# eggsbenedicto/DiffusionRenderer-ComfyUI

Measured on AMD Instinct MI355X. Metric: denoising_steps_per_sec, higher is better.
Workload: dtype bf16; 1 GPU; inverse pass, 57f x 576 x 1024 clip: EDM Euler step = 1 DiT forward (D=4096, 28 blocks, 32 heads) over S=18432 tokens, guidance 0; parallelism=sp1 (token bands; self-attention exchange: none), weights=random-init (hash generator), 7.2e9 params bf16

## Files before the change

diffusionrenderer-comfyui_amd/csrc/gemm256s.hip:

```cpp
#include <stdlib.h>
#include "drn_common.h"
#include "drn_launchers.h"

#ifndef G256S_ABL
#define G256S_ABL 0
#endif
#ifndef G256S_NT
#define G256S_NT 0
#endif
#include "gemm256s_core.h"

#define EPI_PARTIAL 3

template <int EPI, bool PRE = false>
static __device__ __forceinline__ void store_tile(f32x4_t (&acc)[2][4][2][2], bf16_t* C, int64_t M, int64_t N, int64_t ldc,
                                                  const bf16_t* __restrict__ gate, const bf16_t* R, int64_t ldr, int64_t rpb,
                                                  int cbc, int64_t cbs, int64_t m0, int64_t n0, int wr, int wc, int fr, int fq,
                                                  const char* res_lds = nullptr, const char* gate_lds = nullptr) {
    if (G256S_ABL & 8) {
#pragma unroll
        for (int i = 0; i < 2; ++i)
#pragma unroll
            for (int mt = 0; mt < 4; ++mt)
#pragma unroll
                for (int j = 0; j < 2; ++j)
#pragma unroll
                    for (int nt = 0; nt < 2; ++nt) asm volatile("" :: "v"(acc[i][mt][j][nt]));
        return;
    }
    if (EPI == EPI_PARTIAL) {
        float* part = reinterpret_cast<float*>(C);
#pragma unroll
        for (int i = 0; i < 2; ++i)
#pragma unroll
            for (int mt = 0; mt < 4; ++mt) {
                const int64_t m = m0 + i * 128 + wr * 64 + mt * 16 + fr;
                if (m >= M) continue;
#pragma unroll
                for (int j = 0; j < 2; ++j)
#pragma unroll
                    for (int nt = 0; nt < 2; ++nt) {
                        const int64_t n = n0 + j * 128 + wc * 32 + nt * 16 + fq * 4;
                        if (n < N) *reinterpret_cast<f32x4_t*>(part + m * ldc + n) = acc[i][mt][j][nt];
                    }
            }
        return;
    }
    const int64_t c_tile_off = (n0 >> cbc) * cbs + (n0 & ((1ll << cbc) - 1)) - n0;
    asm volatile("" : "+v"(fr), "+v"(fq));
    const int64_t b_tile = (EPI == DRN_EPI_GATE_RES) ? (int64_t)((uint32_t)m0 / (uint32_t)rpb) : 0;
    const bool one_clip = m0 + TB <= (b_tile + 1) * rpb;
#pragma unroll
    for (int i = 0; i < 2; ++i) {
        uint2 g2[4][2][2], r2[4][2][2];
        if (EPI == DRN_EPI_GATE_RES && (G256S_ABL & 64)) {
#pragma unroll
            for (int mt = 0; mt < 4; ++mt)
#pragma unroll
                for (int j = 0; j < 2; ++j)
#pragma unroll
                    for (int nt = 0; nt < 2; ++nt) g2[mt][j][nt] = r2[mt][j][nt] = make_uint2(0x3f803f80u, 0x3f803f80u);
        } else if (EPI == DRN_EPI_GATE_RES && PRE) {
            const uint32_t ra = (uint32_t)((wr * 64 + fr) * 512 + (((wc * 4 + (fq >> 1)) ^ fr) << 4) + (fq & 1) * 8);
#pragma unroll
            for (int mt = 0; mt < 4; ++mt)
#pragma unroll
                for (int j = 0; j < 2; ++j)
#pragma unroll
                    for (int nt = 0; nt < 2; ++nt) {
                        r2[mt][j][nt] = *reinterpret_cast<const uint2*>(res_lds + i * 65536 + mt * 8192 + j * 256 + (ra ^ (nt * 32)));
                        if (mt == 0) {
                            g2[0][j][nt] = *reinterpret_cast<const uint2*>(gate_lds + (j * 128 + wc * 32 + nt * 16 + fq * 4) * 2);
                        } else {
                            g2[mt][j][nt] = g2[0][j][nt];
                        }
                    }
        } else if (EPI == DRN_EPI_GATE_RES) {
#pragma unroll
            for (int mt = 0; mt < 4; ++mt) {
                const int64_t m_raw = m0 + i * 128 + wr * 64 + mt * 16 + fr;
                const int64_t m = m_raw < M ? m_raw : M - 1;
                const int64_t b = one_clip ? b_tile : (int64_t)((uint32_t)m / (uint32_t)rpb);
#pragma unroll
                for (int j = 0; j < 2; ++j)
#pragma unroll
                    for (int nt = 0; nt < 2; ++nt) {
                        const int64_t n = n0 + j * 128 + wc * 32 + nt * 16 + fq * 4;
                        g2[mt][j][nt] = *reinterpret_cast<const uint2*>(gate + b * N + n);
                        r2[mt][j][nt] = *reinterpret_cast<const uint2*>(R + m * ldr + n);
                    }
            }
        }
#pragma unroll
        for (int mt = 0; mt < 4; ++mt) {
            const int64_t m_raw = m0 + i * 128 + wr * 64 + mt * 16 + fr;
            const bool m_ok = m_raw < M;
            const int64_t m = m_ok ? m_raw : M - 1;
#pragma unroll
            for (int j = 0; j < 2; ++j) {
                uint2 o[2];
#pragma unroll
                for (int nt = 0; nt < 2; ++nt) {
                    float v[4];
#pragma unroll
                    for (int r = 0; r < 4; ++r) v[r] = rbf(acc[i][mt][j][nt][r]);
                    if (EPI == DRN_EPI_GELU) {
#pragma unroll
                        for (int r = 0; r < 4; ++r) v[r] = gelu_erf_fast(v[r]);
                    } else if (EPI == DRN_EPI_GATE_RES) {
                        const uint2 gg = g2[mt][j][nt], rr = r2[mt][j][nt];
                        const float g[4] = {bflo(gg.x), bfhi(gg.x), bflo(gg.y), bfhi(gg.y)};
                        const float x[4] = {bflo(rr.x), bfhi(rr.x), bflo(rr.y), bfhi(rr.y)};
#pragma unroll
                        for (int r = 0; r < 4; ++r) v[r] = x[r] + rbf(g[r] * v[r]);
                    }
                    o[nt].x = pack_bf2(v[0], v[1]);
                    o[nt].y = pack_bf2(v[2], v[3]);
                }
                const auto sx = __builtin_amdgcn_permlane16_swap(o[0].x, o[1].x, false, false);
                const auto sy = __builtin_amdgcn_permlane16_swap(o[0].y, o[1].y, false, false);
                const int64_t n8 = n0 + j * 128 + wc * 32 + (fq & 1) * 16 + (fq >> 1) * 8;
                if (G256S_ABL & 128) {
                    asm volatile("" :: "v"(sx[0]), "v"(sy[0]), "v"(sx[1]), "v"(sy[1]));
                } else if (m_ok && n8 < N) {
                    typedef uint32_t u32x4_t __attribute__((ext_vector_type(4)));
                    const u32x4_t val = {sx[0], sy[0], sx[1], sy[1]};
                    u32x4_t* dst = reinterpret_cast<u32x4_t*>(C + m * ldc + n8 + c_tile_off);
                    if (G256S_NT) __builtin_nontemporal_store(val, dst);
                    else *dst = val;
                }
            }
        }
    }
}
#define STORES_PER_TILE 16

template <int EPI, bool PRE = false>
__global__ __launch_bounds__(512, 2) void gemm256s_kernel(const bf16_t* __restrict__ A, const bf16_t* __restrict__ W,
                                                          bf16_t* C, int64_t M, int64_t N, int64_t K, int64_t lda,
                                                          int64_t ldw, int64_t ldc, const bf16_t* __restrict__ gate,
                                                          const bf16_t* R, int64_t ldr, int64_t rpb, int GROUP,
                                                          int abc, int64_t abs_, int cbc, int64_t cbs) {
    if (EPI == EPI_PARTIAL) {
        K /= gridDim.y;
        A += (int64_t)blockIdx.y * K;
        W += (int64_t)blockIdx.y * K;
        C = reinterpret_cast<bf16_t*>(reinterpret_cast<float*>(C) + (int64_t)blockIdx.y * M * ldc);
    }
    THREAD_SETUP();
    int64_t m0, n0;
    tile_of(blockIdx.x, nwg, tiles_m, tiles_n, GROUP, m0, n0);
    const int k_second = min(1, nk - 1);
    int kt = 0;
    if (PRE) {
        (void)gsrc;
        const char* abase = reinterpret_cast<const char*>(A + m0 * lda);
        const char* wbase = reinterpret_cast<const char*>(W + n0 * ldw);
        uint32_t voff[2][2];
#pragma unroll
        for (int p = 0; p < 2; ++p) {
            const int r = (wave * 2 + p) * 8 + (lane >> 3);
            const int c = (lane & 7) ^ ((r >> 1) & 7);
            voff[0][p] = (uint32_t)((r * (int)lda + c * 8) * 2);
            voff[1][p] = (uint32_t)((r * (int)ldw + c * 8) * 2);
        }
#undef DMA
#define DMA(H, KD, S)                                                                                                  \
    do {                                                                                                               \
        const int kt_ = (int)(KD);                                                                                     \
        char* dst_ = smem + H_OFF(S, H) + dma_off;                                                                     \
        const char* sb_ = (H) < 2 ? abase + (((int64_t)((H) & 1) * 128 * lda + A_KOFF(kt_)) << 1)                      \
                                  : wbase + (((int64_t)((H) & 1) * 128 * ldw + (int64_t)kt_ * BK) << 1);               \
        __builtin_amdgcn_global_load_lds((gptr_t)(sb_ + voff[(H) >> 1][0]), (lptr_t)dst_, 16, 0, 0);                   \
        __builtin_amdgcn_global_load_lds((gptr_t)(sb_ + voff[(H) >> 1][1]), (lptr_t)(dst_ + 1024), 16, 0, 0);          \
    } while (0)
        ZERO_ACC();
        PROLOGUE();
        for (; kt + 2 < nk; kt += 2) {
            KSTEP(0, wx, wy, kt + 2, 10, 10, 10, 10);
            KSTEP(1, wy, wx, kt + 3, 10, 10, 10, 10);
        }
        const char* rres = reinterpret_cast<const char*>(R + m0 * ldr + n0);
        uint32_t roff[2];
#pragma unroll
        for (int p = 0; p < 2; ++p) {
            const int rr = wave * 4 + p * 2 + (lane >> 5);
            roff[p] = (uint32_t)((rr * (int)ldr + (((lane & 31) ^ (rr & 15)) << 3)) * 2);
        }
#undef DMA
#define DMA(H, KD, S)                                                                                                  \
    do {                                                                                                               \
        const char* rb_ = rres + (int64_t)(((S) * 4 + (H)) * 32) * ldr * 2;                                            \
        char* dst_ = smem + ((S) * 4 + (H)) * HALF_BYTES + dma_off;                                                    \
        __builtin_amdgcn_global_load_lds((gptr_t)(rb_ + roff[0]), (lptr_t)dst_, 16, 0, 0);                             \
        __builtin_amdgcn_global_load_lds((gptr_t)(rb_ + roff[1]), (lptr_t)(dst_ + 1024), 16, 0, 0);                    \
    } while (0)
        KSTEP(0, wx, wy, 0, 10, 10, 10, 10);
        const char* gbase = reinterpret_cast<const char*>(gate + (int64_t)((uint32_t)m0 / (uint32_t)rpb) * N + n0);
        const uint32_t goff = (uint32_t)((lane & 31) * 16);
        char* gate_lds = smem + 2 * STAGE_BYTES + wave * 1024;
#undef DMA
#define DMA(H, KD, S)                                                                                                  \
    do {                                                                                                               \
        const char* rb_ = rres + (int64_t)(((S) * 4 + (H)) * 32) * ldr * 2;                                            \
        char* dst_ = smem + ((S) * 4 + (H)) * HALF_BYTES + dma_off;                                                    \
        if ((H) == H_W0) __builtin_amdgcn_global_load_lds((gptr_t)(gbase + goff), (lptr_t)gate_lds, 16, 0, 0);         \
        __builtin_amdgcn_global_load_lds((gptr_t)(rb_ + roff[0]), (lptr_t)dst_, 16, 0, 0);                             \
        __builtin_amdgcn_global_load_lds((gptr_t)(rb_ + roff[1]), (lptr_t)(dst_ + 1024), 16, 0, 0);                    \
    } while (0)
        KSTEP(1, wy, wx, 0, 11, 11, 11, 11);
#undef DMA
#define DMA(H, KD, S) GEMM_DMA(H, KD, S)
        asm volatile("s_waitcnt vmcnt(0)" ::: "memory");
        __builtin_amdgcn_s_barrier();
        store_tile<EPI, true>(acc, C, M, N, ldc, gate, R, ldr, rpb, cbc, cbs, m0, n0, wr, wc, fr, fq, smem, gate_lds);
        return;
    }
    SET_SRC(m0, n0);
    ZERO_ACC();
    PROLOGUE();
    for (; kt + 1 < nk; kt += 2) {
        KSTEP(0, wx, wy, min(kt + 2, nk - 1), 10, 10, 10, 10);
        KSTEP(1, wy, wx, min(kt + 3, nk - 1), 10, 10, 10, 10);
    }
    if (kt < nk) KSTEP(0, wx, wy, nk - 1, 10, 10, 10, 10);
    asm volatile("s_waitcnt vmcnt(0)" ::: "memory");
    store_tile<EPI>(acc, C, M, N, ldc, gate, R, ldr, rpb, cbc, cbs, m0, n0, wr, wc, fr, fq);
}

#undef A_OFF
#undef W_OFF
#define A_OFF(S, I) ((S) * 2 * HALF_BYTES + (I) * HALF_BYTES)
#define W_OFF(S, J) (4 * HALF_BYTES + (S) * 2 * HALF_BYTES + (J) * HALF_BYTES)
#define WS_LDS_BYTES (10 * HALF_BYTES)
__global__ __launch_bounds__(512, 2) void gemm256w_kernel(const bf16_t* __restrict__ A, const bf16_t* __restrict__ W,
                                                          float* __restrict__ partial, int64_t M, int64_t N, int64_t K,
                                                          int64_t lda, int64_t ldw, int GROUP) {
    const int abc = 62, cbc = 62;
    const int64_t abs_ = 0, cbs = 0;
    K /= gridDim.y;
    A += (int64_t)blockIdx.y * K;
    W += (int64_t)blockIdx.y * K;
    float* part = partial + (int64_t)blockIdx.y * M * N;
    THREAD_SETUP();
    int64_t m0, n0;
    tile_of(blockIdx.x, nwg, tiles_m, tiles_n, GROUP, m0, n0);
    SET_SRC(m0, n0);
    ZERO_ACC();
#define KCL(k) min((int)(k), nk - 1)
    DMA(H_W0, 0, 0); DMA(H_W1, 0, 0);
    DMA(H_W0, KCL(1), 1); DMA(H_A0, 0, 0); DMA(H_W1, KCL(1), 1); DMA(H_A1, 0, 0);
    DMA(H_W0, KCL(2), 2); DMA(H_A0, KCL(1), 1); DMA(H_W1, KCL(2), 2); DMA(H_A1, KCL(1), 1);
    asm volatile("s_waitcnt vmcnt(12)" ::: "memory");
    __builtin_amdgcn_s_barrier();
#pragma unroll
    for (int nt = 0; nt < 2; ++nt)
#pragma unroll
        for (int ks = 0; ks < 2; ++ks) wx[nt][ks] = LD_W(0, 0, nt, ks);
#pragma unroll
    for (int mt = 0; mt < 4; ++mt)
#pragma unroll
        for (int ks = 0; ks < 2; ++ks) af[mt][ks] = LD_A(0, 0, mt, ks);
    asm volatile("s_waitcnt lgkmcnt(0)" ::: "memory");
    FENCE();
    __builtin_amdgcn_s_barrier();
    FENCE();
    int sw = 0;
#define WSTEP(KT, SA, WA, WB)                                                                                         \
    do {                                                                                                              \
        const int swn_ = sw == 2 ? 0 : sw + 1;                                                                        \
        KSTEP2(SA, (SA) ^ 1, sw, swn_, WA, WB, KCL((KT) + 2), KCL((KT) + 3), 10, 18, 10, 18);                         \
        sw = swn_;                                                                                                    \
    } while (0)
    int kt = 0;
    for (; kt + 1 < nk; kt += 2) {
        WSTEP(kt, 0, wx, wy);
        WSTEP(kt + 1, 1, wy, wx);
    }
    if (kt < nk) WSTEP(kt, 0, wx, wy);
    asm volatile("s_waitcnt vmcnt(0)" ::: "memory");
    store_tile<EPI_PARTIAL>(acc, reinterpret_cast<bf16_t*>(part), M, N, N, nullptr, nullptr, 0, M, cbc, cbs, m0, n0, wr, wc,
                            fr, fq);
}
#undef WSTEP
#undef KCL
#undef A_OFF
#undef W_OFF
#define A_OFF(S, I) ((S) * STAGE_BYTES + (I) * HALF_BYTES)
#define W_OFF(S, J) ((S) * STAGE_BYTES + (2 + (J)) * HALF_BYTES)

#ifndef G256S_PRE_DEFAULT
#define G256S_PRE_DEFAULT 1
#endif
static int g_res_prefetch = G256S_PRE_DEFAULT;
extern "C" int drn_gemm_force_res_prefetch(int on) {
    const int was = g_res_prefetch;
    if (on >= 0) g_res_prefetch = on ? 1 : 0;
    return was;
}

template <int EPI>
static int launch256s(const void* A, const void* W, void* C, int64_t M, int64_t N, int64_t K, int64_t lda, int64_t ldw,
                      int64_t ldc, const void* gate, const void* residual, int64_t ldr, int64_t rpb, hipStream_t st,
                      const int64_t* blk) {
    static bool configured = false;
    if (!configured) {
        hipError_t e = hipFuncSetAttribute(reinterpret_cast<const void*>(&gemm256s_kernel<EPI>),
                                           hipFuncAttributeMaxDynamicSharedMemorySize, 2 * STAGE_BYTES);
        if (e != hipSuccess) return (int)e;
        configured = true;
    }
    const int64_t tiles = ((M + TB - 1) / TB) * ((N + TB - 1) / TB);
    if (tiles >= (1ll << 31) || M >= (1ll << 31)) return DRN_EINVAL;
    if (rpb > M || rpb <= 0) rpb = M;
    static int group = 0;
    if (group == 0) {
        const char* e = getenv("DRN_GEMM_GROUP");
        group = e ? atoi(e) : 4;
        if (group < 1) group = 4;
    }
    if constexpr (EPI == DRN_EPI_GATE_RES) {
        static int pre = -1;
        if (pre < 0) {
            const char* e = getenv("DRN_GEMM_RES_PREFETCH");
            pre = (e && e[0] == '0') ? 0 : 1;
            if (pre && hipFuncSetAttribute(reinterpret_cast<const void*>(&gemm256s_kernel<EPI, true>),
                                           hipFuncAttributeMaxDynamicSharedMemorySize, 2 * STAGE_BYTES + 8192) != hipSuccess) {
                (void)hipGetLastError();
                pre = 0;
            }
        }
        const int64_t nk = K / BK;
        if (pre && g_res_prefetch && M % TB == 0 && N % TB == 0 && rpb % TB == 0 && nk >= 4 && nk % 2 == 0 && residual && gate &&
            ldr % 8 == 0 && ((uintptr_t)residual & 15) == 0 && ((uintptr_t)gate & 15) == 0 && 128 * ldr * 2 < (1ll << 31) && 128 * lda * 2 < (1ll << 31) &&
            128 * ldw * 2 < (1ll << 31)) {
            gemm256s_kernel<EPI, true><<<dim3((unsigned)tiles), dim3(512), 2 * STAGE_BYTES + 8192, st>>>(
                (const bf16_t*)A, (const bf16_t*)W, (bf16_t*)C, M, N, K, lda, ldw, ldc, (const bf16_t*)gate, (const bf16_t*)residual,
                ldr, rpb, group, (int)blk[0], blk[1], (int)blk[2], blk[3]);
            return drn_launch_status();
        }
    }
    gemm256s_kernel<EPI><<<dim3((unsigned)tiles), dim3(512), 2 * STAGE_BYTES, st>>>(
        (const bf16_t*)A, (const bf16_t*)W, (bf16_t*)C, M, N, K, lda, ldw, ldc, (const bf16_t*)gate, (const bf16_t*)residual,
        ldr, rpb, group, (int)blk[0], blk[1], (int)blk[2], blk[3]);
    return drn_launch_status();
}

int drn_gemm256s_partial(const void* A, const void* W, float* partial, int64_t M, int64_t N, int64_t K, int64_t lda, int64_t ldw,
                         int splits, void* stream, bool wring_ok) {
    static bool configured = false;
    if (!configured) {
        hipError_t e = hipFuncSetAttribute(reinterpret_cast<const void*>(&gemm256s_kernel<EPI_PARTIAL>),
                                           hipFuncAttributeMaxDynamicSharedMemorySize, 2 * STAGE_BYTES);
        if (e != hipSuccess) return (int)e;
        configured = true;
    }
    const int64_t tiles = ((M + TB - 1) / TB) * ((N + TB - 1) / TB);
    if (tiles >= 65536 || splits < 1 || splits > 64 || (K / BK) % splits != 0 || M >= (1ll << 31)) return DRN_EINVAL;
    static int wring = -1;
    if (wring < 0) {
        const char* e = getenv("DRN_SPLITK_WRING");
        wring = (e && e[0] == '0') ? 0 : 1;
        if (wring && hipFuncSetAttribute(reinterpret_cast<const void*>(&gemm256w_kernel),
                                         hipFuncAttributeMaxDynamicSharedMemorySize, WS_LDS_BYTES) != hipSuccess) {
            (void)hipGetLastError();
            wring = 0;
        }
    }
    if (wring && wring_ok && K / splits / BK >= 3) {
        gemm256w_kernel<<<dim3((unsigned)tiles, (unsigned)splits), dim3(512), WS_LDS_BYTES, (hipStream_t)stream>>>(
            (const bf16_t*)A, (const bf16_t*)W, partial, M, N, K, lda, ldw, 4);
        return drn_launch_status();
    }
    static const int64_t plain[4] = {62, 0, 62, 0};
    gemm256s_kernel<EPI_PARTIAL><<<dim3((unsigned)tiles, (unsigned)splits), dim3(512), 2 * STAGE_BYTES, (hipStream_t)stream>>>(
        (const bf16_t*)A, (const bf16_t*)W, (bf16_t*)partial, M, N, K, lda, ldw, N, nullptr, nullptr, 0, M, 4,
        (int)plain[0], plain[1], (int)plain[2], plain[3]);
    return drn_launch_status();
}

int drn_gemm256s_dispatch(const void* A, const void* W, void* C, int64_t M, int64_t N, int64_t K, int64_t lda, int64_t ldw,
                          int64_t ldc, int epilogue, const void* gate, const void* residual, int64_t ldr, int64_t rpb,
                          void* stream, const int64_t* blk) {
    hipStream_t st = (hipStream_t)stream;
    switch (epilogue) {
        case DRN_EPI_NONE: return launch256s<DRN_EPI_NONE>(A, W, C, M, N, K, lda, ldw, ldc, gate, residual, ldr, rpb, st, blk);
        case DRN_EPI_GELU: return launch256s<DRN_EPI_GELU>(A, W, C, M, N, K, lda, ldw, ldc, gate, residual, ldr, rpb, st, blk);
        case DRN_EPI_GATE_RES: return launch256s<DRN_EPI_GATE_RES>(A, W, C, M, N, K, lda, ldw, ldc, gate, residual, ldr, rpb, st, blk);
        default: return DRN_EINVAL;
    }
}
```

diffusionrenderer-comfyui_amd/dit_engine.py:

```python
import ctypes
import math
from typing import Dict, NamedTuple, Optional

import torch

from . import native as N
from .host_tables import rope_cos_sin, timestep_sinusoid
from .parallel import ShardPlan, allgather_rows_, alltoall_bands_, alltoall_rows_, group_info, is_process_group, wait_exchange


PRECISIONS = ("bf16", "mxfp8")
ATTENTION_PRECISIONS = ("bf16", "mxfp8")


def _pad_cols(w: torch.Tensor, mult: int) -> torch.Tensor:
    n, k = w.shape
    kp = (k + mult - 1) // mult * mult
    if kp == k:
        return w.contiguous()
    out = torch.zeros((n, kp), dtype=w.dtype, device=w.device)
    out[:, :k] = w
    return out


def _pad_rows(w: torch.Tensor, mult: int) -> torch.Tensor:
    n, k = w.shape
    npad = (n + mult - 1) // mult * mult
    if npad == n:
        return w.contiguous()
    out = torch.zeros((npad, k), dtype=w.dtype, device=w.device)
    out[:n] = w
    return out


class SpRoute(NamedTuple):
    layout: str
    amx: bool
    mx_return: bool = False
    launches: tuple = ()
    first_bands: int = 0
    o_mx: bool = False

    def path(self) -> dict:
        ret = "none" if self.layout == "gather" else ("e4m3" if self.mx_return else "bf16")
        return {"layout": self.layout, "return": ret, "attention": "mxfp8" if self.amx else "bf16"}


def sp_route(D, heads, S, world, exchange, mx, amx_on, fused_mx, mx_return, split_return) -> SpRoute:
    if exchange == "gather":
        amx = bool(amx_on and N.attention_mxfp8_choice(heads, S))
        return SpRoute("gather", amx, o_mx=bool(fused_mx and (amx or N.attention_mx_available())))
    W, rows, hpr = D // world, S // world, heads // world
    if mx:
        slabs = (world > 1 and W >= 256 and W & (W - 1) == 0
                 and N.mx_gemm_plan(rows, 2 * D, D) == 0 and N.mx_gemm_plan(rows, D, D) == 0)
    else:
        slabs = world > 1 and W >= 512 and N.gemm_blocked_ok(rows, 2 * D) and N.gemm_blocked_ok(rows, D)
    amx = bool(amx_on and N.attention_mxfp8_choice(hpr, S))
    mxret = bool(mx and mx_return and (amx or N.attention_mx_available()) and (slabs or world == 1 or (W // 32) % 16 == 0))
    launches = tuple(N.attention_plan(1, hpr, S, S))
    nb = launches[0][1] // rows if len(launches) == 2 and split_return else 0
    return SpRoute("slabs" if slabs else "regroup", amx, mxret, launches, nb)


class HipDiT:
    def __init__(self, net: dict, state_dict: Dict[str, torch.Tensor], device=None, prefix: str = "net.",
                 process_group=None, precision: Optional[str] = None, attention_precision: Optional[str] = None):
        import os
        if attention_precision is None:
            attention_precision = os.environ.get("DRN_ATT_PRECISION", "") or "bf16"
        if attention_precision not in ATTENTION_PRECISIONS:
            raise ValueError(f"unknown attention precision {attention_precision!r}: expected one of {ATTENTION_PRECISIONS}")
        self.attention_precision = attention_precision
        self._amx = attention_precision == "mxfp8"
        if precision is None:
            precision = os.environ.get("DRN_DIT_PRECISION", "") or "bf16"
        if precision not in PRECISIONS:
            raise ValueError(f"unknown DiT precision {precision!r}: expected one of {PRECISIONS}")
        self.precision = precision
        self._mx = precision == "mxfp8"
        if (self._mx or self._amx) and process_group is not None and not is_process_group(process_group):
            which = "precision" if self._mx else "attention_precision"
            raise ValueError(f"{which}='mxfp8' with a process_group that is no torch.distributed.ProcessGroup (sequence parallelism "
                             f"over another transport) is not built yet; got {type(process_group).__name__}")
        self.net = dict(net)
        self.device = torch.device(device) if device is not None else torch.device("cuda")
        self.D = net["model_channels"]
        self.heads = net["num_heads"]
        self.L = net["num_blocks"]
        self.kinds = [k.strip().lower() for k in net["block_config"].split("-")]
        self.pt, self.ps = net["patch_temporal"], net["patch_spatial"]
        self.out_ch = net["out_channels"]
        self.use_ctx = net.get("use_context_embedding", True)
        self.ctx_dim = net["crossattn_emb_channels"]
        self.with_mask = net.get("concat_padding_mask", True)
        if self.D // self.heads != 128:
            raise ValueError("HipDiT kernels are specialised for head_dim 128 (the renderer's only configuration)")
        hidden = int(self.D * net["mlp_ratio"])
        if self._mx and (self.D % 256 or hidden % 256):
            raise ValueError(f"precision='mxfp8' needs model_channels and the MLP width to be multiples of 256 (the MXFP8 GEMM's "
                             f"N and K contract); got {self.D} and {hidden}")
        N.load_library()
        self.pg = process_group
        world = group_info(process_group)[1] if process_group is not None else 1
        mode = os.environ.get("DRN_SP_EXCHANGE", "auto")
        if mode not in ("auto", "a2a", "gather"):
            raise ValueError("DRN_SP_EXCHANGE must be auto, a2a or gather")
        if mode == "a2a" and self.heads % world:
            raise ValueError(f"head all-to-all needs the world size ({world}) to divide the head count ({self.heads})")
        if process_group is None:
            self.exchange = "none"
        elif mode == "auto":
            self.exchange = "none" if world == 1 else ("gather" if self.heads % world else "a2a")
        else:
            self.exchange = mode
        self.world = world
        self._load(state_dict, prefix)
        self._rope_cache = {}
        self._time_cache = {}
        self._ctx_cache = {}
        self._ws = {}
        self._mx_act = {}
        self.trace = None
        self._per_launch = os.environ.get("DRN_PER_LAUNCH", "0") == "1"
        self._mx_fused = self._mx and os.environ.get("DRN_MX_FUSED", "1") != "0"
        self._mx_return = self._mx and os.environ.get("DRN_SP_MX_RETURN", "1") != "0"
        self.sp_path = None
        self._split_return = os.environ.get("DRN_SP_SPLIT_RETURN", "1") != "0"

    def _load(self, sd, p):
        dev, bf = self.device, torch.bfloat16

        def g(name):
            return sd[p + name].to(device=dev, dtype=bf)

        self.w_patch = _pad_cols(g("x_embedder.proj.1.weight"), 64)
        self.kpad = self.w_patch.shape[1]
        self.w_t1 = g("t_embedder.1.linear_1.weight").contiguous().unsqueeze(0)
        self.w_t2 = g("t_embedder.1.linear_2.weight").contiguous().unsqueeze(0)
        self.w_affnorm = g("affline_norm.weight").contiguous()
        self.seq = sd[p + "pos_embedder.seq"]
        self.ctx_table = g("context_embedding.weight") if self.use_ctx else None
        self.w_final = _pad_rows(g("final_layer.linear.weight"), 128)
        self.final_cols = self.out_ch * self.ps * self.ps * self.pt
        self.w_fa1 = g("final_layer.adaLN_modulation.1.weight").contiguous().unsqueeze(0)
        self.w_fa2 = g("final_layer.adaLN_modulation.2.weight").contiguous().unsqueeze(0)

        a1, a2 = [], []
        self.blocks = []
        ca_v, ca_o = [], []
        for i in range(self.L):
            subs = []
            for j, kind in enumerate(self.kinds):
                q = f"blocks.block{i}.blocks.{j}."
                a1.append(g(q + "adaLN_modulation.1.weight"))
                a2.append(g(q + "adaLN_modulation.2.weight"))
                if kind == "fa":
                    a = q + "block.attn."
                    wq, wk, wv = g(a + "to_q.0.weight"), g(a + "to_k.0.weight"), g(a + "to_v.0.weight")
                    if self.exchange == "a2a":
                        W = self.D // self.world
                        wkv = torch.stack([wk.view(self.world, W, -1), wv.view(self.world, W, -1)], 1).reshape(2 * self.D, -1)
                        wqkv = torch.cat([wq, wkv], 0).contiguous()
                    else:
                        wqkv = torch.cat([wq, wk, wv], 0).contiguous()
                    subs.append({"kind": "fa", "wqkv": wqkv,
                                 "qn": g(a + "to_q.1.weight").contiguous(), "kn": g(a + "to_k.1.weight").contiguous(),
                                 "wo": g(a + "to_out.0.weight").contiguous()})
                elif kind == "ca":
                    a = q + "block.attn."
                    subs.append({"kind": "ca", "idx": len(ca_v)})
                    ca_v.append(g(a + "to_v.0.weight"))
                    ca_o.append(g(a + "to_out.0.weight"))
                else:
                    subs.append({"kind": "mlp", "w1": g(q + "block.layer1.weight").contiguous(),
                                 "w2": g(q + "block.layer2.weight").contiguous()})
            self.blocks.append(subs)
        self.n_sites = len(a1)
        self.r = a1[0].shape[0]
        self.w_a1 = torch.cat(a1, 0).contiguous().unsqueeze(0)
        self.w_a2 = torch.stack(a2, 0).contiguous()
        self.n_ca = len(ca_v)
        self.w_cav = torch.stack(ca_v, 0).contiguous() if ca_v else None
        self.w_cao = torch.stack(ca_o, 0).contiguous() if ca_o else None
        self.ca_sites = [i * len(self.kinds) + j for i in range(self.L) for j, k in enumerate(self.kinds) if k == "ca"]
# ... 501 lines not shown
```

diffusionrenderer-comfyui_amd/native.py:

```python
import ctypes
import os
from ctypes import POINTER, Structure, c_char_p, c_double, c_float, c_int, c_int32, c_int64, c_void_p

import torch

_LIB = None
_LIB_NAME = "libdrn.so"

EPI_NONE, EPI_GELU, EPI_GATE_RES = 0, 1, 2
ACT_NONE, ACT_SILU = 0, 1

_P, _I, _L, _F = c_void_p, c_int, c_int64, c_float

SUB_FA, SUB_CA, SUB_MLP = 0, 1, 2


class DitSub(Structure):
    _fields_ = [("kind", c_int32), ("site", c_int32), ("ca_index", c_int32), ("reserved", c_int32),
                ("w_a", c_void_p), ("w_b", c_void_p), ("qn", c_void_p), ("kn", c_void_p),
                ("s_a", c_void_p), ("s_b", c_void_p)]


class DitForwardArgs(Structure):
    _fields_ = [("struct_bytes", c_int64), ("S", c_int64), ("B", c_int64), ("D", c_int64), ("hidden", c_int64),
                ("heads", c_int32), ("n_sub", c_int32), ("subs", POINTER(DitSub)),
                ("shift", c_void_p), ("scale", c_void_p), ("gate", c_void_p),
                ("shift_site_stride", c_int64), ("scale_site_stride", c_int64), ("gate_site_stride", c_int64),
                ("addvec", c_void_p), ("addvec_stride", c_int64), ("cos", c_void_p), ("sin", c_void_p),
                ("P", c_void_p), ("kpad", c_int64), ("w_patch", c_void_p),
                ("final_shift", c_void_p), ("final_scale", c_void_p), ("w_final", c_void_p), ("n_final", c_int64),
                ("X", c_void_p), ("H", c_void_p), ("QKV", c_void_p), ("O", c_void_p), ("U", c_void_p), ("Y", c_void_p),
                ("gemm_ws", c_void_p), ("gemm_ws_bytes", c_int64), ("attn_ws", c_void_p), ("attn_ws_bytes", c_int64),
                ("timer", c_void_p), ("eps", c_float), ("precision", c_int32),
                ("AQ", c_void_p), ("AS", c_void_p), ("act_bytes", c_int64),
                ("mx_fused", c_int32), ("reserved", c_int32), ("UQ", c_void_p), ("US", c_void_p), ("u_act_bytes", c_int64),
                ("attn_precision", c_int32), ("reserved2", c_int32), ("mx_attn", c_void_p), ("mx_attn_bytes", c_int64)]


SIGNATURES = {
    "drn_attention_plan": [_I, _L, _L, POINTER(c_int64)],
    "drn_dit_forward": [POINTER(DitForwardArgs), _P],
    "drn_dit_forward_args_bytes": [],
    "drn_dit_sub_bytes": [],
    "drn_dit_forward_gemm_workspace_bytes": [_L, _L, _L, _L, _L, _L],
    "drn_dit_forward_attn_workspace_bytes": [_L, _I, _L],
    "drn_dit_forward_mx_act_bytes": [_L, _L, _L, _L],
    "drn_dit_forward_mx_gemm_workspace_bytes": [_L, _L, _L, _L],
    "drn_dit_forward_mx_u_bytes": [_L, _L, _L],
    "drn_timer_create": [_I, _I],
    "drn_timer_destroy": [_P],
    "drn_timer_count": [_P],
    "drn_timer_seen": [_P, _I],
    "drn_timer_read": [_P, _I, POINTER(c_int), POINTER(c_float), POINTER(c_double), POINTER(c_double)],
    "drn_abi_version": [],
    "drn_error_string": [_I],
    "drn_gemm_bf16": [_P, _P, _P, _L, _L, _L, _L, _L, _L, _I, _P, _P, _L, _L, _P],
    "drn_gemm_bf16_blocked": [_P, _P, _P, _L, _L, _L, _L, _L, _L, _I, _P, _P, _L, _L, _L, _L, _L, _L, _P],
    "drn_gemm_bf16_splitk": [_P, _P, _P, _L, _L, _L, _L, _L, _L, _I, _P, _P, _L, _L, _I, _P, _P],
    "drn_gemm_splitk_workspace_bytes": [_L, _L, _I],
    "drn_gemm_bf16_f32out": [_P, _P, _P, _L, _L, _L, _L, _L, _P],
    "drn_gemm_bf16_splitk_partials": [_P, _P, _L, _L, _L, _L, _L, _L, _I, _P, _P],
    "drn_splitk_gate_res_ln_modulate": [_P, _I, _P, _P, _P, _P, _P, _P, _L, _L, _L, _F, _P],
    "drn_gemm_splitk_choice": [_L, _L, _L],
    "drn_gemm_tile_choice": [_L, _L],
    "drn_gemm_force_tile": [_I],
    "drn_gemm_force_res_prefetch": [_I],
    "drn_gemm_tall_force_shape": [_I],
    "drn_mx_quant_bf16": [_P, _L, _L, _L, _P, _P, _P],
    "drn_mx_quant_calls": [_I],
    "drn_gemm_mxfp8_gelu_mx": [_P, _P, _P, _P, _P, _P, _L, _L, _L, _L, _P],
    "drn_ln_modulate_mx": [_P, _P, _P, _P, _P, _P, _P, _L, _L, _L, _F, _P],
    "drn_splitk_gate_res_ln_modulate_mx": [_P, _I, _P, _P, _P, _P, _P, _P, _P, _P, _L, _L, _L, _F, _P],
    "drn_attention_bf16_mx": [_P, _P, _P, _P, _P, _P, _I, _I, _L, _L, _L, _L, _L, _L, _L, _L, _L, _L, _F, _P],
    "drn_attention_splitkv_bf16_mx": [_P, _P, _P, _P, _P, _P, _I, _I, _L, _L, _L, _L, _L, _L, _L, _L, _L, _L, _F, _I, _P, _P],
    "drn_attention_mx_available": [],
    "drn_attention_mxfp8_params": [POINTER(c_int), POINTER(c_float), POINTER(c_int)],
    "drn_attention_mxfp8_choice": [_I, _L],
    "drn_attention_mxfp8_force": [_I],
    "drn_qk_norm_rope_mx": [_P, _P, _P, _P, _P, _P, _P, _P, _P, _P, _L, _I, _L, _L, _L, _L, _F, _I, _P],
    "drn_mx_quant_vt": [_P, _P, _P, _I, _I, _L, _L, _L, _P],
    "drn_attention_mxfp8": [_P, _P, _P, _P, _P, _P, _P, _P, _P, _I, _I, _L, _L, _L, _L, _L, _L, _F, _P],
    "drn_attention_splitkv_mxfp8": [_P, _P, _P, _P, _P, _P, _P, _P, _P, _I, _I, _L, _L, _L, _L, _L, _L, _F, _I, _P, _P],
    "drn_dit_forward_mx_attn_bytes": [_L, _L, _L],
    "drn_dit_forward_mx_attn_layout": [_L, _L, _L, POINTER(c_int64)],
    "drn_gemm_mxfp8": [_P, _P, _P, _P, _P, _L, _L, _L, _L, _I, _P, _P, _L, _L, _P],
    "drn_gemm_mxfp8_blocked": [_P, _P, _P, _P, _P, _L, _L, _L, _L, _I, _P, _P, _L, _L, _L, _L, _L, _L, _P],
    "drn_gemm_mxfp8_splitk_choice": [_L, _L, _L],
    "drn_gemm_mxfp8_splitk": [_P, _P, _P, _P, _P, _L, _L, _L, _L, _I, _P, _P, _L, _L, _I, _P, _P],
    "drn_gemm_mxfp8_splitk_partials": [_P, _P, _P, _P, _L, _L, _L, _L, _I, _P, _P],
    "drn_gemm_mxfp8_force_small_m": [_I],
    "drn_gemm_mxfp8_tall_force_shape": [_I],
    "drn_gemv_bf16": [_P, _P, _P, _L, _L, _I, _I, _L, _L, _L, _L, _L, _P, _L, _L, _P, _L, _L, _I, _P],
    "drn_ln_modulate": [_P, _P, _P, _P, _P, _L, _L, _L, _F, _P],
    "drn_ln_force_kernel": [_I],
    "drn_bcast_add": [_P, _P, _L, _L, _L, _P],
    "drn_permute_021": [_P, _P, _L, _L, _L, _P],
    "drn_rmsnorm": [_P, _P, _P, _L, _L, _F, _P],
    "drn_qk_norm_rope": [_P, _P, _P, _P, _P, _P, _L, _I, _L, _L, _L, _L, _F, _P],
    "drn_attention_bf16": [_P, _P, _P, _P, _I, _I, _L, _L, _L, _L, _L, _L, _L, _L, _L, _L, _F, _P],
    "drn_attention_splitkv_bf16": [_P, _P, _P, _P, _I, _I, _L, _L, _L, _L, _L, _L, _L, _L, _L, _L, _F, _I, _P, _P],
    "drn_attention_splitkv_workspace_bytes": [_I, _I, _L, _I],
    "drn_attention_force_shape16": [_I],
    "drn_patchify_concat": [_P, _P, _P, _I, _I, _I, _I, _I, _I, _I, _I, _I, _L, _P],
    "drn_unpatchify": [_P, _L, _P, _I, _I, _I, _I, _I, _I, _I, _P],
    "drn_edm_scale_input": [_P, _P, _L, _F, _P],
    "drn_edm_step": [_P, _P, _P, _L, _F, _F, _F, _F, _P],
    "drn_cfg_combine": [_P, _P, _P, _L, _F, _P],
    "drn_postprocess_u8": [_P, _P, _I, _I, _I, _I, _I, _P],
    "drn_postprocess_window_u8": [_P, _P, _P, _P, _I, _I, _I, _I, _I, _I, _I, _I, _I, _P],
    "drn_env_project": [_P, _I, _P, _P, _P, _P, _I, _I, _I, _F, _P],
    "drn_fit_frames": [_P, _P, _I, _I, _I, _I, _I, _I, _I, _P, _P, _P, _I, _P, _P, _I, _P],
    "drn_fit_frames_u8": [_P, _P, _I, _I, _I, _I, _I, _I, _I, _P, _P, _P, _I, _P, _P, _I, _P],
    "drn_restore_frames_u8": [_P, _P, _I, _I, _I, _I, _I, _I, _I, _P, _P, _I, _P, _P, _I, _P],
    "drn_tile_blend_u8": [_P, _P, _P, _P, _L, _I, _I, _I, _I, _I, _I, _I, _I, _I, _I, _P],
    "drn_latent_tile_gather": [_P, _P, _L, _I, _I, _I, _I, _I, _I, _F, _I, _P],
    "drn_latent_tile_step_join": [_P, _P, _F, _P, _P, _P, _P, _L, _I, _I, _I, _I, _I, _I, _I, _I, _I, _I, _F, _F, _F, _F, _P],
}
_RESTYPES = {"drn_error_string": c_char_p, "drn_attention_splitkv_workspace_bytes": c_int64,
             "drn_gemm_splitk_workspace_bytes": c_int64, "drn_dit_forward_gemm_workspace_bytes": c_int64,
             "drn_dit_forward_attn_workspace_bytes": c_int64, "drn_dit_forward_mx_act_bytes": c_int64,
             "drn_dit_forward_mx_u_bytes": c_int64, "drn_mx_quant_calls": c_int64, "drn_dit_forward_mx_attn_bytes": c_int64,
             "drn_dit_forward_mx_gemm_workspace_bytes": c_int64, "drn_dit_forward_args_bytes": c_int64, "drn_dit_sub_bytes": c_int64, "drn_timer_create": c_void_p, "drn_timer_destroy": None,
             "drn_ln_force_kernel": None, "drn_attention_force_shape16": None}


def library_path() -> str:
    return os.path.join(os.path.dirname(os.path.abspath(__file__)), _LIB_NAME)


def load_library():
    global _LIB
    if _LIB is not None:
        return _LIB
    path = library_path()
    if not os.path.exists(path):
        raise RuntimeError(f"{path} not found: build it with `python __graft_entry__.py` (hipcc --offload-arch=gfx950); "
                           "there is no CPU / eager fallback for the hot path")
    lib = ctypes.CDLL(path)
    for name, argtypes in SIGNATURES.items():
        fn = getattr(lib, name)
        fn.argtypes = argtypes
        fn.restype = _RESTYPES.get(name, c_int)
    if lib.drn_abi_version() != 1:
        raise RuntimeError("libdrn.so ABI version mismatch")
    if lib.drn_dit_forward_args_bytes() != ctypes.sizeof(DitForwardArgs) or lib.drn_dit_sub_bytes() != ctypes.sizeof(DitSub):
        raise RuntimeError("libdrn.so: drn_dit_forward_args / drn_dit_sub layout differs from the ctypes mirror in native.py")
    _LIB = lib
    return lib


def _check(code: int, what: str):
    if code != 0:
        msg = load_library().drn_error_string(code)
        raise RuntimeError(f"{what} failed ({code}): {msg.decode() if msg else '?'}")


def _ptr(t):
    if t is None:
        return None
    assert t.is_cuda, "device tensor required"
    return t.data_ptr()


def _stream():
    return torch.cuda.current_stream().cuda_stream


def _bf16(*ts):
    for t in ts:
        if t is not None:
            assert t.dtype == torch.bfloat16, f"bf16 tensor required, got {t.dtype}"


class KernelTimer:

    def __init__(self, names=("gemm", "attention"), sample_every=1):
        self.names = set(names)
        self.sample_every = max(1, int(sample_every))
        self.counts = {}
        self.records = []
        self._native = None

    def native_handle(self, capacity=8192):
        if not ({"gemm", "attention"} <= self.names):
            return None
        if self._native is None:
            h = load_library().drn_timer_create(capacity, self.sample_every)
            if not h:
                raise RuntimeError("drn_timer_create failed")
            self._native = c_void_p(h)
        return self._native

    def __del__(self):
        if getattr(self, "_native", None) is not None and _LIB is not None:
            _LIB.drn_timer_destroy(self._native)
            self._native = None

    def begin(self, name):
        if name not in self.names:
            return None
        c = self.counts.get(name, 0)
        self.counts[name] = c + 1
        if c % self.sample_every:
            return None
        e = torch.cuda.Event(enable_timing=True)
        e.record()
        return e

    def end(self, name, start, flops, nbytes):
        if start is None:
            return
        e = torch.cuda.Event(enable_timing=True)
        e.record()
        self.records.append((name, start, e, flops, nbytes))

    def summary(self):
        out = {}
        for name, s, e, fl, by in self.records:
            d = out.setdefault(name, {"launches": 0, "ms_total": 0.0, "flops": 0.0, "bytes": 0.0})
            d["launches"] += 1
            d["ms_total"] += s.elapsed_time(e)
            d["flops"] += fl
            d["bytes"] += by
        seen = dict(self.counts)
        if self._native is not None:
            lib = load_library()
            kind, ms, fl, by = c_int(), c_float(), c_double(), c_double()
            for i in range(lib.drn_timer_count(self._native)):
                _check(lib.drn_timer_read(self._native, i, kind, ms, fl, by), "drn_timer_read")
                name = ("gemm", "attention")[kind.value]
# ... 652 lines not shown
```

include/drn.h:

```cpp
#ifndef DRN_H
#define DRN_H

#include <stdint.h>

#ifdef __cplusplus
extern "C" {
#endif

#define DRN_OK 0
#define DRN_EINVAL (-1)

#define DRN_ABI_VERSION 1

#define DRN_EPI_NONE 0
#define DRN_EPI_GELU 1
#define DRN_EPI_GATE_RES 2

#define DRN_ACT_NONE 0
#define DRN_ACT_SILU 1

int drn_abi_version(void);
const char* drn_error_string(int code);

int drn_gemm_bf16(const void* A, const void* W, void* C, int64_t M, int64_t N, int64_t K,
                  int64_t lda, int64_t ldw, int64_t ldc, int epilogue,
                  const void* gate, const void* residual, int64_t ldr, int64_t rows_per_batch,
                  void* stream);

int drn_gemm_bf16_blocked(const void* A, const void* W, void* C, int64_t M, int64_t N, int64_t K,
                          int64_t lda, int64_t ldw, int64_t ldc, int epilogue,
                          const void* gate, const void* residual, int64_t ldr, int64_t rows_per_batch,
                          int64_t a_block_cols, int64_t a_block_stride, int64_t c_block_cols, int64_t c_block_stride,
                          void* stream);

int drn_gemm_bf16_splitk(const void* A, const void* W, void* C, int64_t M, int64_t N, int64_t K,
                         int64_t lda, int64_t ldw, int64_t ldc, int epilogue,
                         const void* gate, const void* residual, int64_t ldr, int64_t rows_per_batch,
                         int splits, void* workspace, void* stream);
int64_t drn_gemm_splitk_workspace_bytes(int64_t M, int64_t N, int splits);
int drn_gemm_bf16_f32out(const void* A, const void* W, float* C, int64_t M, int64_t N, int64_t K, int64_t lda, int64_t ldw, void* stream);

int drn_gemm_bf16_splitk_partials(const void* A, const void* W, int64_t M, int64_t N, int64_t K,
                                  int64_t lda, int64_t ldw, int64_t rows_per_batch, int splits, void* workspace, void* stream);
int drn_gemm_splitk_choice(int64_t M, int64_t N, int64_t K);

int drn_gemm_tile_choice(int64_t M, int64_t N);
void drn_gemm_force_tile(int tile);
int drn_gemm_force_res_prefetch(int on);
int drn_gemm_tall_force_shape(int shape);

int drn_mx_quant_bf16(const void* X, int64_t M, int64_t K, int64_t ldx, void* Q, void* scales, void* stream);
int64_t drn_mx_quant_calls(int reset);
int drn_gemm_mxfp8_gelu_mx(const void* A, const void* SA, const void* W, const void* SW, void* CQ, void* CS, int64_t M, int64_t N,
                           int64_t K, int64_t rows_per_batch, void* stream);
int drn_gemm_mxfp8(const void* A, const void* SA, const void* W, const void* SW, void* C, int64_t M, int64_t N, int64_t K,
                   int64_t ldc, int epilogue, const void* gate, const void* residual, int64_t ldr, int64_t rows_per_batch,
                   void* stream);
int drn_gemm_mxfp8_blocked(const void* A, const void* SA, const void* W, const void* SW, void* C, int64_t M, int64_t N, int64_t K,
                           int64_t ldc, int epilogue, const void* gate, const void* residual, int64_t ldr, int64_t rows_per_batch,
                           int64_t a_block_cols, int64_t a_block_stride, int64_t c_block_cols, int64_t c_block_stride,
                           void* stream);
int drn_gemm_mxfp8_splitk_choice(int64_t M, int64_t N, int64_t K);
int drn_gemm_mxfp8_splitk(const void* A, const void* SA, const void* W, const void* SW, void* C, int64_t M, int64_t N, int64_t K,
                          int64_t ldc, int epilogue, const void* gate, const void* residual, int64_t ldr, int64_t rows_per_batch,
                          int splits, void* workspace, void* stream);
int drn_gemm_mxfp8_splitk_partials(const void* A, const void* SA, const void* W, const void* SW, int64_t M, int64_t N, int64_t K,
                                   int64_t rows_per_batch, int splits, void* workspace, void* stream);
int drn_gemm_mxfp8_force_small_m(int on);
int drn_gemm_mxfp8_tall_force_shape(int shape);

int drn_gemv_bf16(const void* x, const void* W, void* y, int64_t N, int64_t K,
                  int groups, int batch,
                  int64_t x_gstride, int64_t x_bstride, int64_t w_gstride,
                  int64_t y_gstride, int64_t y_bstride,
                  const void* add, int64_t add_gstride, int64_t add_bstride,
                  const void* mul, int64_t mul_gstride, int64_t mul_bstride,
                  int act, void* stream);

int drn_ln_modulate(void* x, const void* add_vec, const void* shift, const void* scale, void* h,
                    int64_t rows, int64_t D, int64_t rows_per_batch, float eps, void* stream);
int drn_ln_modulate_mx(void* x, const void* add_vec, const void* shift, const void* scale, void* h, void* hq, void* hs,
                       int64_t rows, int64_t D, int64_t rows_per_batch, float eps, void* stream);
int drn_splitk_gate_res_ln_modulate(const void* partials, int splits, void* x, const void* gate, const void* add_vec,
                                    const void* shift, const void* scale, void* h, int64_t rows, int64_t D,
                                    int64_t rows_per_batch, float eps, void* stream);
int drn_splitk_gate_res_ln_modulate_mx(const void* partials, int splits, void* x, const void* gate, const void* add_vec,
                                       const void* shift, const void* scale, void* h, void* hq, void* hs, int64_t rows, int64_t D,
                                       int64_t rows_per_batch, float eps, void* stream);
void drn_ln_force_kernel(int which);

int drn_bcast_add(void* x, const void* vec, int64_t rows, int64_t D, int64_t rows_per_batch, void* stream);

int drn_permute_021(const void* x, void* y, int64_t A, int64_t B, int64_t C, void* stream);

int drn_rmsnorm(const void* x, const void* w, void* y, int64_t rows, int64_t D, float eps, void* stream);

int drn_qk_norm_rope(void* q, void* k, const void* wq, const void* wk, const void* cos, const void* sin,
                     int64_t tokens, int heads, int64_t ldq, int64_t ldk, int64_t tokens_per_batch,
                     int64_t pos_offset, float eps, void* stream);

int drn_attention_bf16(const void* q, const void* k, const void* v, void* o,
                       int batch, int heads, int64_t Sq, int64_t Sk,
                       int64_t ldq, int64_t ldk, int64_t ldv, int64_t ldo,
                       int64_t bsq, int64_t bsk, int64_t bsv, int64_t bso,
                       float scale, void* stream);

void drn_attention_force_shape16(int on);

int drn_attention_splitkv_bf16(const void* q, const void* k, const void* v, void* o,
                               int batch, int heads, int64_t Sq, int64_t Sk,
                               int64_t ldq, int64_t ldk, int64_t ldv, int64_t ldo,
                               int64_t bsq, int64_t bsk, int64_t bsv, int64_t bso,
                               float scale, int nsplit, void* workspace, void* stream);
int64_t drn_attention_splitkv_workspace_bytes(int batch, int heads, int64_t Sq, int nsplit);

int drn_attention_bf16_mx(const void* q, const void* k, const void* v, void* o, void* oq, void* os,
                          int batch, int heads, int64_t Sq, int64_t Sk,
                          int64_t ldq, int64_t ldk, int64_t ldv, int64_t ldo,
                          int64_t bsq, int64_t bsk, int64_t bsv, int64_t bso,
                          float scale, void* stream);
int drn_attention_splitkv_bf16_mx(const void* q, const void* k, const void* v, void* o, void* oq, void* os,
                                  int batch, int heads, int64_t Sq, int64_t Sk,
                                  int64_t ldq, int64_t ldk, int64_t ldv, int64_t ldo,
                                  int64_t bsq, int64_t bsk, int64_t bsv, int64_t bso,
                                  float scale, int nsplit, void* workspace, void* stream);
int drn_attention_mx_available(void);

int drn_attention_mxfp8_params(int* key_tile, float* rescale_thr, int* pexp);
int drn_attention_mxfp8_choice(int heads, int64_t S);
int drn_attention_mxfp8_force(int on);
int drn_qk_norm_rope_mx(void* q, void* k, const void* wq, const void* wk, const void* cos, const void* sin,
// ... 149 lines not shown
```

Baseline: 3.687 steps/s.

## Replace GELU epilogue math with a bf16 lookup table staged in LDS

Builds a 65536-entry bf16 GELU lookup table once per device and, in the 256x256 GEMM's GELU epilogue, DMAs it into shared memory after the K loop. Each output is then rounded to bf16 and mapped through the table instead of evaluating erf-based GELU per element. This removes transcendental ALU work from the MLP up-projection epilogue. In exchange it adds a 128KB table load per tile and LDS gather lookups with possible bank conflicts, and it drops the bounds check on the store path, relying on the M and N tile-divisibility guard at launch.

```diff
diff --git a/diffusionrenderer-comfyui_amd/csrc/gemm256s.hip b/diffusionrenderer-comfyui_amd/csrc/gemm256s.hip
--- a/diffusionrenderer-comfyui_amd/csrc/gemm256s.hip
+++ b/diffusionrenderer-comfyui_amd/csrc/gemm256s.hip
@@ -1,4 +1,5 @@
 #include <stdlib.h>
+#include <mutex>
 #include "drn_common.h"
 #include "drn_launchers.h"
 
@@ -11,6 +12,19 @@
 #include "gemm256s_core.h"
 
 #define EPI_PARTIAL 3
+
+static __device__ __forceinline__ uint32_t gelu_table2(const char* table_lds, uint32_t w) {
+    uint32_t wl = w & 0xffffu;
+    asm("" : "+v"(wl));
+    const uint32_t lo = *reinterpret_cast<const uint16_t*>(table_lds + (wl << 1));
+    const uint32_t hi = *reinterpret_cast<const uint16_t*>(table_lds + ((w >> 16) << 1));
+    return lo | (hi << 16);
+}
+__global__ void gelu_table_kernel(bf16_t* __restrict__ table) {
+    const uint32_t i = blockIdx.x * blockDim.x + threadIdx.x;
+    if (i < 65536u) table[i] = f2bf(gelu_erf_fast(bf2f((bf16_t)i)));
+}
+#define GELU_TABLE_BYTES (65536 * 2)
 
 template <int EPI, bool PRE = false>
 static __device__ __forceinline__ void store_tile(f32x4_t (&acc)[2][4][2][2], bf16_t* C, int64_t M, int64_t N, int64_t ldc,
@@ -95,12 +109,18 @@
         for (int mt = 0; mt < 4; ++mt) {
             const int64_t m_raw = m0 + i * 128 + wr * 64 + mt * 16 + fr;
             const bool m_ok = m_raw < M;
-            const int64_t m = m_ok ? m_raw : M - 1;
+            const int64_t m = (m_ok || (EPI == DRN_EPI_GELU && PRE)) ? m_raw : M - 1;
 #pragma unroll
             for (int j = 0; j < 2; ++j) {
                 uint2 o[2];
 #pragma unroll
                 for (int nt = 0; nt < 2; ++nt) {
+                    if (EPI == DRN_EPI_GELU && PRE) {
+                        const f32x4_t a = acc[i][mt][j][nt];
+                        o[nt].x = gelu_table2(res_lds, pack_bf2(a[0], a[1]));
+                        o[nt].y = gelu_table2(res_lds, pack_bf2(a[2], a[3]));
+                        continue;
+                    }
                     float v[4];
 #pragma unroll
                     for (int r = 0; r < 4; ++r) v[r] = rbf(acc[i][mt][j][nt][r]);
@@ -122,7 +142,7 @@
                 const int64_t n8 = n0 + j * 128 + wc * 32 + (fq & 1) * 16 + (fq >> 1) * 8;
                 if (G256S_ABL & 128) {
                     asm volatile("" :: "v"(sx[0]), "v"(sy[0]), "v"(sx[1]), "v"(sy[1]));
-                } else if (m_ok && n8 < N) {
+                } else if ((EPI == DRN_EPI_GELU && PRE) || (m_ok && n8 < N)) {
                     typedef uint32_t u32x4_t __attribute__((ext_vector_type(4)));
                     const u32x4_t val = {sx[0], sy[0], sx[1], sy[1]};
                     u32x4_t* dst = reinterpret_cast<u32x4_t*>(C + m * ldc + n8 + c_tile_off);
@@ -179,6 +199,26 @@
         for (; kt + 2 < nk; kt += 2) {
             KSTEP(0, wx, wy, kt + 2, 10, 10, 10, 10);
             KSTEP(1, wy, wx, kt + 3, 10, 10, 10, 10);
+        }
+        if constexpr (EPI == DRN_EPI_GELU) {
+            const char* tbase = reinterpret_cast<const char*>(gate) + dma_off;
+            const uint32_t toff = (uint32_t)(lane * 16);
+#undef DMA
+#define DMA(H, KD, S)                                                                                                  \
+    do {                                                                                                               \
+        const char* tb_ = tbase + ((S) * 4 + (H)) * HALF_BYTES;                                                        \
+        char* dst_ = smem + ((S) * 4 + (H)) * HALF_BYTES + dma_off;                                                    \
+        __builtin_amdgcn_global_load_lds((gptr_t)(tb_ + toff), (lptr_t)dst_, 16, 0, 0);                                \
+        __builtin_amdgcn_global_load_lds((gptr_t)(tb_ + toff + 1024), (lptr_t)(dst_ + 1024), 16, 0, 0);                \
+    } while (0)
+            KSTEP(0, wx, wy, 0, 10, 10, 10, 10);
+            KSTEP(1, wy, wx, 0, 10, 10, 10, 10);
+#undef DMA
+#define DMA(H, KD, S) GEMM_DMA(H, KD, S)
+            asm volatile("s_waitcnt vmcnt(0)" ::: "memory");
+            __builtin_amdgcn_s_barrier();
+            store_tile<EPI, true>(acc, C, M, N, ldc, nullptr, nullptr, 0, rpb, cbc, cbs, m0, n0, wr, wc, fr, fq, smem, nullptr);
+            return;
         }
         const char* rres = reinterpret_cast<const char*>(R + m0 * ldr + n0);
         uint32_t roff[2];
@@ -299,6 +339,49 @@
     return was;
 }
 
+static int g_gelu_table_on = 1;
+extern "C" int drn_gemm_force_gelu_table(int on) {
+    const int was = g_gelu_table_on;
+    if (on >= 0) g_gelu_table_on = on ? 1 : 0;
+    return was;
+}
+
+#define DRN_MAX_DEVICES 64
+static bf16_t* g_gelu_table[DRN_MAX_DEVICES];
+static std::mutex g_gelu_table_mutex;
+extern "C" int drn_gemm_gelu_table_build(void* stream) {
+    int dev = -1;
+    hipError_t e = hipGetDevice(&dev);
+    if (e != hipSuccess) {
+        (void)hipGetLastError();
+        return (int)e;
+    }
+    if (dev < 0 || dev >= DRN_MAX_DEVICES) return DRN_EINVAL;
+    std::lock_guard<std::mutex> lock(g_gelu_table_mutex);
+    if (g_gelu_table[dev]) return DRN_OK;
+    bf16_t* t = nullptr;
+    e = hipMalloc(reinterpret_cast<void**>(&t), GELU_TABLE_BYTES);
+    if (e != hipSuccess) {
+        (void)hipGetLastError();
+        return (int)e;
+    }
+    gelu_table_kernel<<<dim3(256), dim3(256), 0, (hipStream_t)stream>>>(t);
+    e = hipGetLastError();
+    if (e == hipSuccess) e = hipStreamSynchronize((hipStream_t)stream);
+    if (e != hipSuccess) {
+        (void)hipFree(t);
+        return (int)e;
+    }
+    g_gelu_table[dev] = t;
+    return DRN_OK;
+}
+static const bf16_t* gelu_table_here() {
+    int dev = -1;
+    if (hipGetDevice(&dev) != hipSuccess || dev < 0 || dev >= DRN_MAX_DEVICES) return nullptr;
+    std::lock_guard<std::mutex> lock(g_gelu_table_mutex);
+    return g_gelu_table[dev];
+}
+
 template <int EPI>
 static int launch256s(const void* A, const void* W, void* C, int64_t M, int64_t N, int64_t K, int64_t lda, int64_t ldw,
                       int64_t ldc, const void* gate, const void* residual, int64_t ldr, int64_t rpb, hipStream_t st,
@@ -340,6 +423,28 @@
             return drn_launch_status();
         }
     }
+    if constexpr (EPI == DRN_EPI_GELU) {
+        static int lut = -1;
+        if (lut < 0) {
+            const char* e = getenv("DRN_GEMM_GELU_TABLE");
+            lut = (e && e[0] == '0') ? 0 : 1;
+            if (lut && hipFuncSetAttribute(reinterpret_cast<const void*>(&gemm256s_kernel<EPI, true>),
+                                           hipFuncAttributeMaxDynamicSharedMemorySize, 2 * STAGE_BYTES) != hipSuccess) {
+                (void)hipGetLastError();
+                lut = 0;
+            }
+        }
+        const int64_t nk = K / BK;
+        if (lut && g_gelu_table_on && M % TB == 0 && N % TB == 0 && nk >= 4 && nk % 2 == 0 && 128 * lda * 2 < (1ll << 31) &&
+            128 * ldw * 2 < (1ll << 31)) {
+            if (const bf16_t* table = gelu_table_here()) {
+                gemm256s_kernel<EPI, true><<<dim3((unsigned)tiles), dim3(512), 2 * STAGE_BYTES, st>>>(
+                    (const bf16_t*)A, (const bf16_t*)W, (bf16_t*)C, M, N, K, lda, ldw, ldc, table, nullptr, 0, rpb, group,
+                    (int)blk[0], blk[1], (int)blk[2], blk[3]);
+                return drn_launch_status();
+            }
+        }
+    }
     gemm256s_kernel<EPI><<<dim3((unsigned)tiles), dim3(512), 2 * STAGE_BYTES, st>>>(
         (const bf16_t*)A, (const bf16_t*)W, (bf16_t*)C, M, N, K, lda, ldw, ldc, (const bf16_t*)gate, (const bf16_t*)residual,
         ldr, rpb, group, (int)blk[0], blk[1], (int)blk[2], blk[3]);
diff --git a/diffusionrenderer-comfyui_amd/dit_engine.py b/diffusionrenderer-comfyui_amd/dit_engine.py
--- a/diffusionrenderer-comfyui_amd/dit_engine.py
+++ b/diffusionrenderer-comfyui_amd/dit_engine.py
@@ -101,6 +101,9 @@
             raise ValueError(f"precision='mxfp8' needs model_channels and the MLP width to be multiples of 256 (the MXFP8 GEMM's "
                              f"N and K contract); got {self.D} and {hidden}")
         N.load_library()
+        if self.device.type == "cuda":
+            with torch.cuda.device(self.device):
+                N._check(N.load_library().drn_gemm_gelu_table_build(None), "drn_gemm_gelu_table_build")
         self.pg = process_group
         world = group_info(process_group)[1] if process_group is not None else 1
         mode = os.environ.get("DRN_SP_EXCHANGE", "auto")
diff --git a/diffusionrenderer-comfyui_amd/native.py b/diffusionrenderer-comfyui_amd/native.py
--- a/diffusionrenderer-comfyui_amd/native.py
+++ b/diffusionrenderer-comfyui_amd/native.py
@@ -65,6 +65,8 @@
     "drn_gemm_tile_choice": [_L, _L],
     "drn_gemm_force_tile": [_I],
     "drn_gemm_force_res_prefetch": [_I],
+    "drn_gemm_gelu_table_build": [_P],
+    "drn_gemm_force_gelu_table": [_I],
     "drn_gemm_tall_force_shape": [_I],
     "drn_mx_quant_bf16": [_P, _L, _L, _L, _P, _P, _P],
     "drn_mx_quant_calls": [_I],
@@ -146,6 +148,7 @@
     if lib.drn_dit_forward_args_bytes() != ctypes.sizeof(DitForwardArgs) or lib.drn_dit_sub_bytes() != ctypes.sizeof(DitSub):
         raise RuntimeError("libdrn.so: drn_dit_forward_args / drn_dit_sub layout differs from the ctypes mirror in native.py")
     _LIB = lib
+    lib.drn_gemm_gelu_table_build(None)
     return lib
 
 
diff --git a/include/drn.h b/include/drn.h
--- a/include/drn.h
+++ b/include/drn.h
@@ -47,6 +47,8 @@
 int drn_gemm_tile_choice(int64_t M, int64_t N);
 void drn_gemm_force_tile(int tile);
 int drn_gemm_force_res_prefetch(int on);
+int drn_gemm_gelu_table_build(void* stream);
+int drn_gemm_force_gelu_table(int on);
 int drn_gemm_tall_force_shape(int shape);
 
 int drn_mx_quant_bf16(const void* X, int64_t M, int64_t K, int64_t ldx, void* Q, void* scales, void* stream);
```

Result: no change. 3.688 steps/s, median of 2 (+0.0%).
